# gitshitou/aclswarm

Measured on AMD Instinct MI355X. Metric: swarm assignment+control solves/sec (N=100) at 1/2/4/8 MI355X; % HBM roofline, higher is better.
Workload: dtype f64

## Files before the change

aclswarm_amd/_lib.py:

```python
import ctypes as ct
import os

import numpy as np

LIB_PATH = os.environ.get("ACLSWARM_AMD_LIB") or os.path.join(
    os.path.dirname(os.path.abspath(__file__)), "lib", "libaclswarm_amd.so")

ACL_OK = 0

FLAG_VALID = 0x01
FLAG_AGREE = 0x02
FLAG_CHANGED = 0x04
FLAG_NONFINITE = 0x08
FLAG_BAD_INPUT = 0x10
FLAG_CA_ACTIVE = 0x20
ABI_VERSION = 11
FLAG_FRAGILE = 0x40
FRAGILE_MARGIN = 1e-6

STATUS_DTYPE = np.dtype([("flags", "<u4"), ("eff_rounds", "<u2"),
                         ("rounds", "<u2"), ("n_invalid", "<u2"),
                         ("n_ca", "<u2"), ("margin", "<f4")])

EXPORTS = (
# ... 118 lines not shown
    _fields_ = [("B", ct.c_int32), ("fidx", ct.c_void_p), ("q", ct.c_void_p),
                ("vel", ct.c_void_p), ("P", ct.c_void_p), ("flush", ct.c_void_p),
                ("est", ct.c_void_p), ("ring_u", ct.c_void_p), ("ring_ca", ct.c_void_p),
                ("step0", ct.c_int32), ("steps", ct.c_int32), ("q_hist", ct.c_void_p),
                ("vel_hist", ct.c_void_p), ("u_hist", ct.c_void_p), ("ca_hist", ct.c_void_p), ("P_hist", ct.c_void_p),
                ("workspace", ct.c_void_p), ("cntrl", CntrlGains), ("safety", SafetyParams),
                ("ep", EpisodeParams)]


class TrialParams(ct.Structure):
    _fields_ = [("ep", EpisodeParams), ("tick_rate", ct.c_int32), ("settle_steps", ct.c_int32),
                ("hover_wait", ct.c_double), ("assignment_timeout", ct.c_double),
                ("formation_received_wait", ct.c_double), ("converged_wait", ct.c_double),
                ("gridlock_timeout", ct.c_double), ("trial_timeout", ct.c_double),
                ("alpha", ct.c_double)]


TRIAL_HOVERING, TRIAL_WAITING, TRIAL_FLYING, TRIAL_IN_FORMATION = 3, 4, 5, 6
TRIAL_GRIDLOCK, TRIAL_COMPLETE, TRIAL_TERMINATE = 7, 8, 9

TRIAL_STATUS_DTYPE = np.dtype([(k, "<i4") for k in (
    "state", "last_state", "timer_ticks", "formation", "ticks", "received", "logging",
    "commit", "next_auction", "conv_len", "conv_head", "grid_len", "grid_head", "log_init",
    "t_start", "t_grid", "done_step")] + [("n_auctions", "<u2"), ("n_invalid", "<u2"),
                                          ("n_skipped", "<u2"), ("n_disagree", "<u2"),
                                          ("per_vehicle", "<i4")])


class TrialArgs(ct.Structure):
    _fields_ = [("B", ct.c_int32), ("K", ct.c_int32)] + [
        (k, ct.c_void_p) for k in ("fseq", "fidx", "q", "vel", "P", "flush", "ts", "ctl_on",
                                   "ring_u", "ring_ca", "posf", "dist", "t_conv", "t_avoid",
                                   "n_assign")] + [
        ("step0", ct.c_int32), ("steps", ct.c_int32)] + [
        (k, ct.c_void_p) for k in ("q_hist", "vel_hist", "u_hist", "ca_hist", "ctl_hist",
                                   "P_hist", "state_hist", "workspace")] + [
        ("cntrl", CntrlGains), ("safety", SafetyParams), ("tp", TrialParams)]


HUNG_BAD_INPUT = 0x01
HUNG_NONFINITE = 0x02
HUNG_CMP_INVALID = 0x04

_lib = None


def lib():
    global _lib
    if _lib is not None:
        return _lib
    if not os.path.exists(LIB_PATH):
        raise RuntimeError(
            f"aclswarm_amd: native library {LIB_PATH} is missing. Build it with "
            "`python -m aclswarm_amd.build` (hipcc --offload-arch=gfx950).")
    import torch
    L = ct.CDLL(LIB_PATH)
    VP, I32, I64, SZ = ct.c_void_p, ct.c_int32, ct.c_int64, ct.c_size_t
    L.acl_default_cntrl_gains.argtypes = [ct.POINTER(CntrlGains)]
    L.acl_default_safety_params.argtypes = [ct.POINTER(SafetyParams)]
    L.acl_default_admm_params.argtypes = [ct.POINTER(AdmmParams)]
    L.acl_formations_init.argtypes = [ct.POINTER(Formations), I32, I32]
    L.acl_formations_init.restype = None
    L.acl_max_vehicles.restype = I32
    L.acl_abi_version.restype = I32
    if L.acl_abi_version() != ABI_VERSION:
        raise RuntimeError(f"aclswarm_amd: {LIB_PATH} has ABI {L.acl_abi_version()}, this "
                           f"package expects {ABI_VERSION}: rebuild (python -m aclswarm_amd.build)")
    L.acl_solve_workspace_bytes.argtypes = [I32, I32]
    L.acl_solve_workspace_bytes.restype = ct.c_size_t
    L.acl_solve_batch.argtypes = [ct.POINTER(Formations), ct.POINTER(SolveArgs), VP]
    L.acl_solve_batch.restype = ct.c_int
    L.acl_count_edges.argtypes = [I32, VP]
    L.acl_count_edges.restype = I64
    L.acl_pack_adjacency.argtypes = [I32, VP, VP]
    L.acl_pack_adjacency.restype = ct.c_int
    L.acl_pack_gains.argtypes = [I32, VP, VP, VP]
    L.acl_pack_gains.restype = ct.c_int
    L.acl_gain_planes.argtypes = [I32, VP, VP]
    L.acl_gain_planes.restype = I32
    L.acl_pack_gains_planes.argtypes = [I32, VP, VP, I32, VP]
    L.acl_pack_gains_planes.restype = ct.c_int
    L.acl_tile_gains.argtypes = [ct.POINTER(Formations), VP, VP]
    L.acl_swarm_stats.argtypes = [VP, I32, VP, VP, VP]
    L.acl_swarm_stats.restype = I32
    L.acl_tile_gains.restype = ct.c_int
    L.acl_admm_solve_batch.argtypes = [I32, I32, VP, VP, VP, VP, ct.POINTER(AdmmParams), VP]
    L.acl_admm_solve_batch.restype = ct.c_int
    L.acl_control_batch.argtypes = [ct.POINTER(Formations), ct.POINTER(ControlArgs), VP]
    L.acl_control_batch.restype = ct.c_int
    L.acl_default_episode_params.argtypes = [ct.POINTER(EpisodeParams)]
    L.acl_default_episode_params.restype = None
    L.acl_episode_workspace_bytes.argtypes = [I32, I32]
    L.acl_episode_workspace_bytes.restype = SZ
    L.acl_episode_batch.argtypes = [ct.POINTER(Formations), ct.POINTER(EpisodeArgs), VP]
    L.acl_episode_batch.restype = ct.c_int
    L.acl_default_trial_params.argtypes = [ct.POINTER(TrialParams)]
    L.acl_default_trial_params.restype = None
    L.acl_trial_workspace_bytes.argtypes = [I32, I32]
    L.acl_trial_workspace_bytes.restype = SZ
    L.acl_trial_init.argtypes = [ct.POINTER(TrialArgs), I32, VP]
    L.acl_trial_init.restype = ct.c_int
    L.acl_trial_batch.argtypes = [ct.POINTER(Formations), ct.POINTER(TrialArgs), VP]
    L.acl_trial_batch.restype = ct.c_int
    L.acl_generate_formation_groups.argtypes = [I32, I32, VP, I32, ct.c_double, ct.c_double,
                                                ct.c_double, ct.c_double, I64, VP, VP, VP,
                                                VP, VP]
    L.acl_generate_formation_groups.restype = ct.c_int
    L.acl_hungarian_batch.argtypes = [ct.POINTER(Formations), ct.POINTER(HungarianArgs), VP]
    L.acl_hungarian_batch.restype = ct.c_int
    L.acl_cbaa_step_batch.argtypes = [ct.POINTER(Formations), ct.POINTER(CbaaStepArgs), VP]
    L.acl_cbaa_step_batch.restype = ct.c_int
    L.acl_vehicle_start_batch.argtypes = [ct.POINTER(Formations), ct.POINTER(VehicleStartArgs),
                                          VP]
    L.acl_vehicle_start_batch.restype = ct.c_int
    L.acl_fleet_workspace_bytes.argtypes = [I32, I32, I32]
    L.acl_fleet_workspace_bytes.restype = SZ
    L.acl_fleet_auction_batch.argtypes = [ct.POINTER(Formations), ct.POINTER(FleetAuctionArgs),
                                          VP]
    L.acl_fleet_auction_batch.restype = ct.c_int
    L.acl_write_assignment_log.argtypes = [ct.c_char_p, I32, VP, VP, VP, VP, VP, VP]
    L.acl_write_assignment_log.restype = ct.c_int
    L.acl_read_assignment_log.argtypes = [ct.c_char_p, ct.POINTER(I32), VP, VP, VP, VP, VP, VP]
    L.acl_read_assignment_log.restype = ct.c_int
    L.acl_device_count.restype = I32
    L.acl_set_device.argtypes = [I32]
    L.acl_set_device.restype = ct.c_int
    L.acl_malloc.argtypes = [ct.POINTER(VP), SZ]
    L.acl_malloc.restype = ct.c_int
    L.acl_free.argtypes = [VP]
    L.acl_free.restype = ct.c_int
    for fn in ("acl_memcpy_h2d", "acl_memcpy_d2h"):
        getattr(L, fn).argtypes = [VP, VP, SZ, VP]
        getattr(L, fn).restype = ct.c_int
    L.acl_memset.argtypes = [VP, ct.c_int, SZ, VP]
    L.acl_memset.restype = ct.c_int
    L.acl_stream_synchronize.argtypes = [VP]
    L.acl_stream_synchronize.restype = ct.c_int
    L.acl_last_error.restype = ct.c_char_p
    L.acl_internal_kernel_timing.argtypes = [ct.c_int]
    L.acl_internal_kernel_timing.restype = None
    L.acl_internal_kernel_times.argtypes = [ct.POINTER(ct.c_double), ct.POINTER(ct.c_int)]
    L.acl_internal_kernel_times.restype = ct.c_int
    L.acl_internal_admm_flop_counter.argtypes = [VP]
    L.acl_internal_admm_flop_counter.restype = None
    if hasattr(L, "acl_internal_admm_mem_cap"):
        L.acl_internal_admm_mem_cap.argtypes = [SZ]
        L.acl_internal_admm_mem_cap.restype = None
    L.acl_internal_psd_project.argtypes = [ct.c_int, ct.c_int, VP, ct.c_double, VP, ct.c_int,
                                           ct.POINTER(ct.c_int)]
    L.acl_internal_psd_project.restype = ct.c_int
    if hasattr(L, "acl_internal_price_sweep"):
        L.acl_internal_price_sweep.argtypes = [VP, VP, VP, ct.c_int]
        L.acl_internal_price_sweep.restype = ct.c_int
    _lib = L
    return L


def check(rc, what="aclswarm_amd"):
    if rc != ACL_OK:
        msg = lib().acl_last_error().decode(errors="replace")
        raise RuntimeError(f"{what} failed (code {rc}): {msg}")


def default_episode_params():
    e = EpisodeParams()
    lib().acl_default_episode_params(ct.byref(e))
    return e


def default_trial_params():
    t = TrialParams()
    lib().acl_default_trial_params(ct.byref(t))
    return t


def default_gains():
    g = CntrlGains()
    lib().acl_default_cntrl_gains(ct.byref(g))
    return g


def default_safety():
    s = SafetyParams()
    lib().acl_default_safety_params(ct.byref(s))
    return s


def default_admm_params():
    a = AdmmParams()
    lib().acl_default_admm_params(ct.byref(a))
    return a
```

aclswarm_amd/csrc/auction.hip:

```cpp
#include <hip/hip_runtime.h>
#include <stdint.h>

#include "../../include/aclswarm_amd.h"
#include "common.h"
#include "control_dev.h"
#include "control_params.h"
#include "pair_fused.h"
#include "umeyama_dev.h"

namespace acl_amd {

#ifndef ACL_AUCTION_LEVELS
#define ACL_AUCTION_LEVELS 4
#endif
constexpr int kAL = ACL_AUCTION_LEVELS;

__host__ __device__ inline int a16(int x) { return (x + 15) & ~15; }

struct ALayout {
  int C, pq, adjF, items;
  int A, p, qf, out;
  int T, TS;
  int vadj, Pin, Ptin, itm, valid, H, misc, dummy, W1, total;
};
// ... 1112 lines not shown
      P.P_out[(size_t)b * n + v] = (uint16_t)jj;
      validv[v] = valid0;
      if (jj != Pin[v]) misc[M_CHANGED] = 1;
    }
  } else {
    for (int v = wave; v < n; v += kAW) {
      const unsigned char* row = T + v * TS;
      bool ismine[NC];
#pragma unroll
      for (int c = 0; c < NC; ++c) {
        const int jj = lane + 64 * c;
        ismine[c] = (jj < n) && (row[jj] == v);
      }
      int mine = -1;
#pragma unroll
      for (int c = NC - 1; c >= 0; --c) {
        const unsigned long long mm = __ballot(ismine[c]);
        if (mm) mine = 64 * c + __ffsll((long long)mm) - 1;
      }
      const bool valid = row_valid(row) && mine >= 0;
      const int adopted = valid ? mine : Pin[v];
      if (lane == 0) {
        validv[v] = valid;
        if (!valid) atomicAdd(&misc[M_NINV], 1);
        if (adopted != Pin[v]) misc[M_CHANGED] = 1;
        P.P_out[(size_t)b * n + v] = (uint16_t)adopted;
      }
    }
  }
  if (P.who) {
    for (int k = tid; k < n * n; k += kAB) {
      const int v = k / n, jj = k - v * n;
      const int w = T[v * TS + jj];
      P.who[(size_t)b * n * n + k] = (w >= n) ? (uint16_t)0xFFFF : (uint16_t)w;
    }
  }
  __syncthreads();
  stamp_phase(P, b, tid, 5);

  const int ninv = misc[M_NINV];
  const bool allvalid = ninv == 0;
  const bool uniform = (allvalid && misc[M_AGREE]) || (ninv == n && !rowsm);
  const int ptv = (uniform && tid < n) ? (allvalid ? T[tid] : Ptin[tid]) : 0;
  {
    uint16_t* wsPt = reinterpret_cast<uint16_t*>(P.ws + P.W.pt) + (size_t)b * n;
    if (tid == 0) P.ws[P.W.mode + b] = uniform ? 0 : 1;
    if (uniform) {
      for (int jj = tid; jj < n; jj += kAB) wsPt[jj] = allvalid ? T[jj] : Ptin[jj];
    } else {
      uint16_t* rows = reinterpret_cast<uint16_t*>(P.ws + P.W.rows) + (size_t)b * n * n;
      for (int k = tid; k < n * n; k += kAB) {
        const int v = k / n, jj = k - v * n;
        rows[k] = validv[v] ? T[v * TS + jj]
                  : rowsm ? P.P_rows[(size_t)b * n * n + k] : Ptin[jj];
      }
      for (int v = tid; v < n; v += kAB) P.ws[P.W.vvalid + (size_t)b * n + v] = validv[v];
    }
    if (tid == 0) {
      acl_swarm_status_t st = {};
      uint32_t fl = 0;
      if (allvalid) fl |= ACL_SWARM_VALID;
      if (misc[M_AGREE]) fl |= ACL_SWARM_AGREE;
      if (misc[M_CHANGED]) fl |= ACL_SWARM_CHANGED;
      if (nonfinite) fl |= ACL_SWARM_NONFINITE;
      const double g = !MG ? -1.0 : nonfinite ? 0.0 : __longlong_as_double((long long)*margw);
      if (MG && g < ACL_FRAGILE_MARGIN) fl |= ACL_SWARM_FRAGILE;
      st.flags = fl;
      st.eff_rounds = (uint16_t)eff;
      st.rounds = (uint16_t)(2 * n);
      st.n_invalid = (uint16_t)ninv;
      st.margin = (float)g;
      P.status[b] = st;
    }
  }
  stamp_phase(P, b, tid, 6);

  if constexpr (FUSE) {
    if (!uniform) return;
#ifdef ACL_EXP_SKIP_GAIN
    return;
#endif
    __syncthreads();
    const FusedLayout GL = make_fused_layout(n, kAW);
    if (tid < n) reinterpret_cast<uint16_t*>(smem + GL.Pt)[tid] = (uint16_t)ptv;
    KCtlParams* pc = (KCtlParams*)((const __attribute__((address_space(4))) char*)
                                       __builtin_amdgcn_kernarg_segment_ptr() +
                                   offsetof(SolveParams, ctl));
    asm volatile("" : "+s"(pc));
    if (!ACL_FUSED_PREFETCH) fused_prefetch(*pc, b, f, tid, fpre);
    if (ACL_CTL_PRIO || ACL_CBAA_PRIO) __builtin_amdgcn_s_setprio(ACL_CTL_PRIO);
    pair_gain_fused<kAW, GM>(pc, b, f, smem, tid, kAB, fpre);
    stamp_phase(P, b, tid, 7);
  }
  stamp_rt(P, b, tid, kStampRt1);
}

__global__ void price_sweep_kernel(const double* x, float* fast, float* ieee, int m) {
  const int i = blockIdx.x * blockDim.x + threadIdx.x;
  if (i < m) {
    fast[i] = acl_price(x[i]);
    ieee[i] = (float)(1.0 / (sqrt(x[i]) + 1e-8));
  }
}

static int auction_lds(int n, bool fuse) {
  const int a = make_alayout(n).total;
  if (!fuse) return a;
  const int kAW = n <= 32 ? 2 : (n <= 64 ? 4 : 8);
  const int g = make_fused_layout(n, kAW).total;
  return a > g ? a : g;
}

template <bool FUSE, bool GM, bool MG>
static hipError_t launch_auction_t(const SolveParams& P, int nb, hipStream_t stream) {
  static PerDeviceOnce once;
  const hipError_t ea = once.run([] {
    for (const void* k : {(const void*)auction_kernel<1, 128, FUSE, GM, MG>,
                          (const void*)auction_kernel<1, 256, FUSE, GM, MG>,
                          (const void*)auction_kernel<2, 512, FUSE, GM, MG>}) {
      const hipError_t e =
          hipFuncSetAttribute(k, hipFuncAttributeMaxDynamicSharedMemorySize, 160 * 1024);
      if (e != hipSuccess) return e;
    }
    return hipSuccess;
  });
  if (ea != hipSuccess) return ea;
  if (P.n > 64)
    hipLaunchKernelGGL((align_kernel<2>), dim3(nb), dim3(64), make_align_layout(P.n).total, stream,
                       P);
  const int lds = auction_lds(P.n, FUSE);
  if (P.n <= 32)
    hipLaunchKernelGGL((auction_kernel<1, 128, FUSE, GM, MG>), dim3(nb), dim3(128), lds, stream, P);
  else if (P.n <= 64)
    hipLaunchKernelGGL((auction_kernel<1, 256, FUSE, GM, MG>), dim3(nb), dim3(256), lds, stream, P);
  else
    hipLaunchKernelGGL((auction_kernel<2, 512, FUSE, GM, MG>), dim3(nb), dim3(512), lds, stream, P);
  return hipGetLastError();
}

hipError_t launch_auction(const SolveParams& P, int nb, hipStream_t stream, bool fuse) {
  const bool mg = !P.skip_margin;
  if (!fuse)
    return mg ? launch_auction_t<false, false, true>(P, nb, stream)
              : launch_auction_t<false, false, false>(P, nb, stream);
  if (P.ctl.gate_margin)
    return mg ? launch_auction_t<true, true, true>(P, nb, stream)
              : launch_auction_t<true, true, false>(P, nb, stream);
  return mg ? launch_auction_t<true, false, true>(P, nb, stream)
            : launch_auction_t<true, false, false>(P, nb, stream);
}

}

extern "C" int acl_internal_price_sweep(const double* x, float* fast, float* ieee, int m) {
  if (m <= 0) return 0;
  hipLaunchKernelGGL(acl_amd::price_sweep_kernel, dim3((m + 255) / 256), dim3(256), 0, 0, x, fast,
                     ieee, m);
  return hipDeviceSynchronize() == hipSuccess ? 0 : 1;
}
```

aclswarm_amd/csrc/pair_fused.h:

```cpp
#pragma once

#include "control_dev.h"

#ifndef ACL_DIAG_NOPAIR
#define ACL_DIAG_NOPAIR 0
#endif
#ifndef ACL_DIAG_NOLOADS
#define ACL_DIAG_NOLOADS 0
#endif
#ifndef ACL_DIAG_NOLOOP
#define ACL_DIAG_NOLOOP 0
#endif

namespace acl_amd {

struct FusedLayout {
  int pt, adj, etab, rowb, Pt, Pinv, acc, atab, cst, nearb, clf, vel, flags, gmw, caw, total;
};

enum { FC_K1XY, FC_K2XY, FC_K1Z, FC_K2Z, FC_TXY, FC_TZ, FC_WIN, FC_THR2, FC_N };

__host__ __device__ inline FusedLayout make_fused_layout(int n, int kW) {
  const int nb = (n + 7) >> 3, R = 8 * nb;
  FusedLayout L;
  int o = 0;
  L.pt = o;    o = cal16(o + R * 64);
  L.adj = o;   o = cal16(o + R * 2 * 8);
  L.etab = o;  o = cal16(o + R * nb * 4);
  L.rowb = o;  o = cal16(o + (R + 1) * 4);
  L.Pt = o;    o = cal16(o + n * 2);
  L.Pinv = o;  o = cal16(o + n * 2);
  L.acc = o;   o = cal16(o + kW * R * 3 * 8);
  L.atab = o;  o = cal16(o + ACL_ATAB_N * 8);
  L.cst = o;   o = cal16(o + FC_N * 8);
  L.nearb = o; o = cal16(o + 4 * 4);
  L.clf = o;   o = cal16(o + R * 4);
  L.vel = o;   o = cal16(o + n * 24);
  L.flags = o; o = cal16(o + 4);
  L.gmw = o;   o = o + 8;
  L.caw = o;   o = cal16(o + 4);
  L.total = o;
  return L;
}

struct Rec5 {
  double a[5];
};

__device__ __forceinline__ void load_rec5(__amdgpu_buffer_rsrc_t grs, int voff, Rec5& R) {
  const auto r0 = __builtin_amdgcn_raw_buffer_load_b128(grs, voff, 0, 0);
  const auto r1 = __builtin_amdgcn_raw_buffer_load_b128(grs, voff, 16, 0);
  const auto r2 = __builtin_amdgcn_raw_buffer_load_b64(grs, voff, 32, 0);
  __builtin_memcpy(&R.a[0], &r0, 16);
  __builtin_memcpy(&R.a[2], &r1, 16);
  __builtin_memcpy(&R.a[4], &r2, 8);
}

constexpr unsigned long long kTileUpIncl = 0x80C0E0F0F8FCFEFFull;
constexpr unsigned long long kTileUpStrict = kTileUpIncl & ~0x8040201008040201ull;
constexpr unsigned long long kColLanes = 0x000000FF00FF00FFull;

__device__ __forceinline__ double f64_of(unsigned lo, unsigned hi) {
  return __longlong_as_double((long long)(((unsigned long long)hi << 32) | lo));
}

__device__ __forceinline__ double col3_neg(double a, double b, double c3) {
  const unsigned long long ua = (unsigned long long)__double_as_longlong(a);
  const unsigned long long ub = (unsigned long long)__double_as_longlong(b);
  const auto s0 = __builtin_amdgcn_permlane32_swap((unsigned)ua, (unsigned)ub, false, false);
  const auto s1 = __builtin_amdgcn_permlane32_swap((unsigned)(ua >> 32), (unsigned)(ub >> 32),
                                                   false, false);
  const double p = f64_of(s0[0], s1[0]) + f64_of(s0[1], s1[1]);
  const double cc = swap_sum<32>(c3);
  const unsigned long long up = (unsigned long long)__double_as_longlong(p);
  const unsigned long long uc = (unsigned long long)__double_as_longlong(cc);
  const auto t0 = __builtin_amdgcn_permlane16_swap((unsigned)up, (unsigned)uc, false, false);
  const auto t1 = __builtin_amdgcn_permlane16_swap((unsigned)(up >> 32), (unsigned)(uc >> 32),
                                                   false, false);
  const double qn = -(f64_of(t0[0], t1[0]) + f64_of(t0[1], t1[1]));
  return qn + dpp_f64_all<0x128>(qn);
}

__device__ __forceinline__ double fcst(const double* cst, int k) {
  return *((const volatile __attribute__((address_space(3))) double*)(cst) + k);
}

typedef const __attribute__((address_space(4))) CtlParams KCtlParams;

__device__ __forceinline__ acl_cntrl_gains_t kgains(KCtlParams& P) {
  acl_cntrl_gains_t g;
  g.K1_xy = P.g.K1_xy; g.K2_xy = P.g.K2_xy; g.K1_z = P.g.K1_z; g.K2_z = P.g.K2_z;
  g.e_xy_thr = P.g.e_xy_thr; g.e_z_thr = P.g.e_z_thr; g.kp = P.g.kp; g.kd = P.g.kd;
  return g;
}

__device__ __forceinline__ acl_safety_params_t ksafety(KCtlParams& P) {
  acl_safety_params_t s;
  s.max_vel_xy = P.s.max_vel_xy; s.max_vel_z = P.s.max_vel_z;
  s.d_avoid_thresh = P.s.d_avoid_thresh; s.r_keep_out = P.s.r_keep_out;
  return s;
}

struct FusedPre {
  double q0, q1, q2, v0, v1, v2, px, py, pz;
  unsigned long long a0, a1;
};

__device__ __forceinline__ void fused_prefetch(KCtlParams& P, int b, int f, int tid,
                                               FusedPre& X) {
  const int n = P.n;
  X.q0 = X.q1 = X.q2 = X.v0 = X.v1 = X.v2 = X.px = X.py = X.pz = 0.0;
  X.a0 = X.a1 = 0ull;
  if (tid < n) {
    const int NWg = (n + 63) >> 6;
    const unsigned long long lastmask = (n & 63) ? ((1ull << (n & 63)) - 1ull) : ~0ull;
    const double* gq = P.q + ((size_t)b * n + tid) * 3;
    const double* gv = P.vel + ((size_t)b * n + tid) * 3;
    const double* gp = P.p + ((size_t)f * n + tid) * 3;
    const uint64_t* ga = P.adj + ((size_t)f * n + tid) * NWg;
    X.q0 = gq[0]; X.q1 = gq[1]; X.q2 = gq[2];
    X.v0 = gv[0]; X.v1 = gv[1]; X.v2 = gv[2];
    X.px = gp[0]; X.py = gp[1]; X.pz = gp[2];
    X.a0 = ga[0];
    if (NWg > 1) X.a1 = ga[1] & lastmask;
    else X.a0 &= lastmask;
  }
}

template <int kW, bool GM>
__device__ __forceinline__ void pair_gain_fused(KCtlParams* Pp, int b, int f,
                                                unsigned char* smem, int tid, int nthreads,
                                                const FusedPre& X) {
  KCtlParams& P = *Pp;
  const int n = P.n;
  const int nb = (n + 7) >> 3, R = 8 * nb;
  const FusedLayout L = make_fused_layout(n, kW);
  const int lane = tid & 63;
  const int wave = __builtin_amdgcn_readfirstlane(tid >> 6);

  double* pt = reinterpret_cast<double*>(smem + L.pt);
  unsigned long long* adjF = reinterpret_cast<unsigned long long*>(smem + L.adj);
  unsigned* etab = reinterpret_cast<unsigned*>(smem + L.etab);
  int* rowb = reinterpret_cast<int*>(smem + L.rowb);
  const uint16_t* Pt = reinterpret_cast<const uint16_t*>(smem + L.Pt);
  uint16_t* Pinv = reinterpret_cast<uint16_t*>(smem + L.Pinv);
  double* acc = reinterpret_cast<double*>(smem + L.acc);
  double* atab = reinterpret_cast<double*>(smem + L.atab);
  double* cst = reinterpret_cast<double*>(smem + L.cst);
  unsigned* nearb = reinterpret_cast<unsigned*>(smem + L.nearb);
  unsigned* clf = reinterpret_cast<unsigned*>(smem + L.clf);
  double* velv = reinterpret_cast<double*>(smem + L.vel);
  unsigned* flags = reinterpret_cast<unsigned*>(smem + L.flags);
  unsigned long long& gmw = *reinterpret_cast<unsigned long long*>(smem + L.gmw);
  unsigned* caw = reinterpret_cast<unsigned*>(smem + L.caw);
  double* qs = acc;

  for (int k = tid; k < ACL_ATAB_N; k += nthreads) atab[k] = ACL_ATAB_AT(k);
  if (GM && tid == 0) gmw = (unsigned long long)__double_as_longlong(__builtin_inf());
  if (tid == 0) {
    *caw = 0u;
    *flags = 0u;
  }
  if (tid < 4) nearb[tid] = 0u;
  for (int k = tid; k < R; k += nthreads) clf[k] = 0u;
  if (tid < FC_N) {
    const double thr_hi = P.s.d_avoid_thresh * (1.0 + 0x1p-40);
    const double v[FC_N] = {P.g.K1_xy, P.g.K2_xy, P.g.K1_z, P.g.K2_z,
                            P.g.e_xy_thr, P.g.e_z_thr, ACL_GATE_WINDOW, thr_hi * thr_hi};
    double x = v[0];
#pragma unroll
    for (int k = 1; k < FC_N; ++k) x = tid == k ? v[k] : x;
    cst[tid] = x;
  }
  {
    bool qbad = false;
    if (tid < n) {
      const int v = tid;
      qs[3 * v] = X.q0;
      qs[3 * v + 1] = X.q1;
      qs[3 * v + 2] = X.q2;
      velv[3 * v] = X.v0;
      velv[3 * v + 1] = X.v1;
      velv[3 * v + 2] = X.v2;
      qbad = !(__builtin_isfinite(X.q0) && __builtin_isfinite(X.q1) && __builtin_isfinite(X.q2));
    }
    if (tid < R) {
      const int i = tid;
      double row[5] = {0.0, 0.0, 0.0, 0.0, 0.0};
      if (i < n) {
        Pinv[Pt[i]] = (uint16_t)i;
        const double x = X.px, y = X.py, z = X.pz;
        row[0] = x;
        row[1] = y;
        row[2] = z;
        row[3] = x * x + y * y;
        row[4] = z * z;
      }
      pt[8 * i + 3] = row[0];
      reinterpret_cast<double4*>(pt + 8 * i)[1] = make_double4(row[1], row[2], row[3], row[4]);
      adjF[2 * i] = X.a0;
      adjF[2 * i + 1] = X.a1;
    }
    if (__any(qbad) && lane == 0) atomicOr(flags, 1u);
  }
  __syncthreads();
  if (tid < R) {
    const int i = tid;
    double q0 = 0.0, q1 = 0.0, q2 = 0.0;
    if (i < n) {
      const int v = Pt[i];
      q0 = qs[3 * v];
      q1 = qs[3 * v + 1];
      q2 = qs[3 * v + 2];
    }
    pt[8 * i] = q0;
    pt[8 * i + 1] = q1;
    pt[8 * i + 2] = q2;
  }
  if (wave == 0) {
    int base = 0;
    for (int i0 = 0; i0 < R; i0 += 64) {
      const int i = i0 + lane;
      const int cnt = (i < R) ? __popcll(adjF[2 * i]) + __popcll(adjF[2 * i + 1]) : 0;
      int x = cnt;
      x += __builtin_amdgcn_update_dpp(0, x, 0x111, 0xF, 0xF, true);
      x += __builtin_amdgcn_update_dpp(0, x, 0x112, 0xF, 0xF, true);
      x += __builtin_amdgcn_update_dpp(0, x, 0x114, 0xF, 0xF, true);
      x += __builtin_amdgcn_update_dpp(0, x, 0x118, 0xF, 0xF, true);
      x += __builtin_amdgcn_update_dpp(0, x, 0x142, 0xA, 0xF, false);
      x += __builtin_amdgcn_update_dpp(0, x, 0x143, 0xC, 0xF, false);
      if (i < R) rowb[i] = base + x - cnt;
      base += __builtin_amdgcn_readlane(x, 63);
    }
    if (lane == 0) rowb[R] = base;
  }
  __syncthreads();
  const unsigned nbm = (65536u + (unsigned)nb - 1u) / (unsigned)nb;
  for (int k = tid; k < R * nb; k += nthreads) {
    const int i = (int)(((unsigned)k * nbm) >> 16), J = k - i * nb;
    const int w = J >> 3, sh = (8 * J) & 63;
    const unsigned long long word = adjF[2 * i + w];
    const unsigned below = (unsigned)__popcll(sh ? (word & ((1ull << sh) - 1ull)) : 0ull) +
                           (w ? (unsigned)__popcll(adjF[2 * i]) : 0u);
    etab[k] = ((unsigned)rowb[i] + below) << 8 | (unsigned)((word >> sh) & 0xFFull);
  }
  for (int k = tid; k < kW * R * 3; k += nthreads) acc[k] = 0.0;
  const bool qfin = (*flags & 1u) == 0u;
  __syncthreads();

  double gmxy = __builtin_inf(), gmz = __builtin_inf();
  if (wave < kW) {
    const int E = __builtin_amdgcn_readfirstlane(rowb[R]);
    const double* G = P.gains + 5 * P.gain_off[f];
    const __amdgpu_buffer_rsrc_t grs =
        __builtin_amdgcn_make_buffer_rsrc((void*)G, (short)0, 5 * E * 8, 0x00020000);
    const int r = lane >> 3, c = lane & 7;
    const int colk = 3 * c + ((lane >> 4) == 0 ? 0 : ((lane >> 4) == 1 ? 2 : 1));
    const int NT = nb * (nb + 1) / 2;
    const int t0 = (wave * NT) / kW, t1 = ACL_DIAG_NOLOOP ? t0 : ((wave + 1) * NT) / kW;
    double* myacc = acc + wave * R * 3;

    int I = 0, J = 0;
    if (t0 < t1) {
      int rem = t0;
      while (rem >= nb - I) {
        rem -= nb - I;
        ++I;
      }
      J = I + rem;
    }
    auto rec_mask = [&](unsigned x, int s, bool diag, unsigned long long up) {
      return __ballot((x >> s) & 1u) & (diag ? up : ~0ull);
    };
    auto rec_load = [&](unsigned x, int s, unsigned long long m, Rec5& R) {
      const unsigned e = (x >> 8) + (unsigned)__popc(x & ((1u << s) - 1u));
#if ACL_DIAG_NOLOADS
      const double d = (double)(lanebit_u64(m) ? (e & 7u) : 0u) * 0.125;
      R.a[0] = d; R.a[1] = -d; R.a[2] = d; R.a[3] = d; R.a[4] = -d;
#else
      load_rec5(grs, lanebit_u64(m) ? (int)__umul24(e, 40u) : 0x40000000, R);
#endif
    };
    Rec5 X, Y;
    unsigned long long mx = 0ull, my = 0ull;
    if (t0 < t1) {
      const unsigned xij = etab[__umul24(8 * I + r, nb) + J], xji = etab[__umul24(8 * J + c, nb) + I];
      mx = rec_mask(xij, c, I == J, kTileUpIncl);
      my = rec_mask(xji, r, I == J, kTileUpStrict);
      rec_load(xij, c, mx, X);
      rec_load(xji, r, my, Y);
    }
    double ra0 = 0.0, ra1 = 0.0, ra2 = 0.0;
#pragma unroll 1
    for (int t = t0; t < t1; ++t) {
#pragma clang fp contract(fast)
      int In = I, Jn = J;
      if (++Jn == nb) {
        ++In;
        Jn = In;
      }
      const bool more = t + 1 < t1;
      unsigned xijn = 0u, xjin = 0u;
      if (more) {
        xijn = etab[__umul24(8 * In + r, nb) + Jn];
        xjin = etab[__umul24(8 * Jn + c, nb) + In];
      }
      const int i = 8 * I + r, j = 8 * J + c;
      const double4* pi = reinterpret_cast<const double4*>(pt + 8 * i);
      const double4* pj = reinterpret_cast<const double4*>(pt + 8 * j);
      const double4 ai = pi[0], aj = pj[0];
      const double q0 = aj.x - ai.x, q1 = aj.y - ai.y, q2 = aj.z - ai.z;
      const double s2 = pair_s2(q0, q1);
      {
        const int nr = n - 8 * I, nc = n - 8 * J;
        const unsigned long long rows = nr >= 8 ? ~0ull : ((1ull << (8 * nr)) - 1ull);
        const unsigned long long cols =
            (nc >= 8 ? 0xFFull : ((1ull << nc) - 1ull)) * 0x0101010101010101ull;
        const unsigned long long vm = rows & cols & (I == J ? kTileUpStrict : ~0ull);
        const unsigned long long nm = __ballot(!(s2 > fcst(cst, FC_THR2))) & vm;
        if (nm) {
          if (lanebit_u64(nm)) {
            atomicOr(&nearb[i >> 5], 1u << (i & 31));
            atomicOr(&nearb[j >> 5], 1u << (j & 31));
          }
        }
      }
      const unsigned long long many = mx | my;
      double Fxy = 0.0, Fz = 0.0;
      if (!ACL_DIAG_NOPAIR && lanebit_u64(many)) {
        const double4 bi = pi[1], bj = pj[1];
        const double pix = ai.w, piy = bi.x, piz = bi.y, pjx = aj.w, pjy = bj.x, pjz = bj.y;
        double e_xy, e_z;
        pair_e(q0, q1, q2, bi.z, bj.z, bi.w, bj.w, pix, piy, piz, pjx, pjy, pjz, s2, e_xy, e_z);
        bool gxy, gz;
        gate_decide_t<GM>(fcst(cst, FC_TXY), fcst(cst, FC_TZ), fcst(cst, FC_WIN), e_xy, e_z, q0,
                          q1, q2, bi.z, bj.z, bi.w, bj.w, pix, piy, piz, pjx, pjy, pjz, gxy, gz,
                          gmxy, gmz);
#if ACL_DIAG_NOATAN
        if (gxy) Fxy = fcst(cst, FC_K1XY) * (fcst(cst, FC_K2XY) * e_xy);
        if (gz) Fz = fcst(cst, FC_K1Z) * (fcst(cst, FC_K2Z) * e_z);
#else
        if (gxy) Fxy = fcst(cst, FC_K1XY) * ACL_GAIN_ATAN(fcst(cst, FC_K2XY) * e_xy, atab);
        if (gz) Fz = fcst(cst, FC_K1Z) * ACL_GAIN_ATAN(fcst(cst, FC_K2Z) * e_z, atab);
#endif
      }
      const double f0 = Fxy * q0, f1 = Fxy * q1, f2 = Fz * q2;
      if (lanebit_u64(mx)) {
        if (qfin) {
          ra0 += X.a[1] * q1 + (X.a[0] * q0 + f0);
          ra1 += X.a[3] * q1 + (X.a[2] * q0 + f1);
          ra2 += X.a[4] * q2 + f2;
        } else {
          ra0 += ((X.a[0] * q0 + X.a[1] * q1) + 0.0 * q2) + f0;
          ra1 += ((X.a[2] * q0 + X.a[3] * q1) + 0.0 * q2) + f1;
          ra2 += ((0.0 * q0 + 0.0 * q1) + X.a[4] * q2) + f2;
        }
      }
      unsigned long long mxn = 0ull, myn = 0ull;
      if (more) {
        mxn = rec_mask(xijn, c, In == Jn, kTileUpIncl);
        rec_load(xijn, c, mxn, X);
      }
      double ct0 = 0.0, ct1 = 0.0, ct2 = 0.0;
      if (lanebit_u64(my)) {
        if (qfin) {
          ct0 = Y.a[1] * q1 + (Y.a[0] * q0 + f0);
          ct1 = Y.a[3] * q1 + (Y.a[2] * q0 + f1);
          ct2 = Y.a[4] * q2 + f2;
        } else {
          ct0 = ((Y.a[0] * q0 + Y.a[1] * q1) + 0.0 * q2) + f0;
          ct1 = ((Y.a[2] * q0 + Y.a[3] * q1) + 0.0 * q2) + f1;
          ct2 = ((0.0 * q0 + 0.0 * q1) + Y.a[4] * q2) + f2;
        }
      }
      if (more) {
        myn = rec_mask(xjin, r, In == Jn, kTileUpStrict);
        rec_load(xjin, r, myn, Y);
      }
      {
        const double cs = col3_neg(ct0, ct1, ct2);
        if (lanebit_u64(kColLanes)) unsafeAtomicAdd(myacc + 24 * J + colk, cs);
      }
      if (!more || In != I) {
        ra0 += dpp_f64_all<0xB1>(ra0); ra1 += dpp_f64_all<0xB1>(ra1); ra2 += dpp_f64_all<0xB1>(ra2);
        ra0 += dpp_f64_all<0x4E>(ra0); ra1 += dpp_f64_all<0x4E>(ra1); ra2 += dpp_f64_all<0x4E>(ra2);
        ra0 += dpp_f64_all<0x141>(ra0); ra1 += dpp_f64_all<0x141>(ra1); ra2 += dpp_f64_all<0x141>(ra2);
        if (c == 0) {
          double* a = myacc + 3 * i;
          unsafeAtomicAdd(a, ra0);
          unsafeAtomicAdd(a + 1, ra1);
          unsafeAtomicAdd(a + 2, ra2);
        }
        ra0 = ra1 = ra2 = 0.0;
      }
      I = In;
      J = Jn;
      mx = mxn;
      my = myn;
    }
    if (GM) {
      const acl_cntrl_gains_t g = kgains(P);
      gate_margin_reduce(&gmw, gate_margin_of(g, gmxy, gmz));
    }
  }
  __syncthreads();
  if (GM && tid == 0) P.gate_margin[b] = __longlong_as_double((long long)gmw);
  if (nearb[0] | nearb[1] | nearb[2] | nearb[3]) {
    const double thr = P.s.d_avoid_thresh;
    const double thr_hi = thr * (1.0 + 0x1p-40);
    const double thr2hi = thr_hi * thr_hi;
    const int per = nthreads / n;
    const int v = tid % n, j0 = tid / n;
    if (j0 < per) {
      const int i = Pinv[v];
      if ((nearb[i >> 5] >> (i & 31)) & 1u) {
        const double qv0 = pt[8 * i], qv1 = pt[8 * i + 1];
        bool c = false;
        for (int k = j0; k < n; k += per) {
          const double dx = pt[8 * k] - qv0, dy = pt[8 * k + 1] - qv1;
          const double d2 = dx * dx + dy * dy;
          if (k != i && !(d2 > thr2hi)) c |= !(sqrt(d2) > thr);
        }
        if (c) clf[v] = 1u;
      }
    }
    __syncthreads();
  }

  {
    const acl_cntrl_gains_t g = kgains(P);
    const acl_safety_params_t sp = ksafety(P);
    const int NW = (n + 63) >> 6;
    for (int v = tid; v < n; v += nthreads) {
      const int i = Pinv[v];
      const int deg = __popcll(adjF[2 * i]) + __popcll(adjF[2 * i + 1]);
      double s0 = 0.0, s1 = 0.0, s2 = 0.0;
      for (int w = 0; w < kW; ++w) {
        const double* a = acc + (w * R + i) * 3;
        s0 += a[0];
        s1 += a[1];
        s2 += a[2];
      }
      double cmd0 = g.kp * s0, cmd1 = g.kp * s1, cmd2 = g.kp * s2;
      if (deg) {
        const double* gv = velv + 3 * v;
        const double cn = (double)deg;
        cmd0 += cn * (g.kd * (-gv[0]));
        cmd1 += cn * (g.kd * (-gv[1]));
        cmd2 += cn * (g.kd * (-gv[2]));
      }
      double* gu = P.u + ((size_t)b * n + v) * 3;
      gu[0] = cmd0;
      gu[1] = cmd1;
      gu[2] = cmd2;
      saturate(sp, cmd0, cmd1, cmd2);
      const bool close = clf[v] != 0u;
      if (P.u_safe) {
        double* o = P.u_safe + ((size_t)b * n + v) * 3;
        o[0] = cmd0;
        o[1] = cmd1;
        o[2] = cmd2;
      }
      if (P.ca_flag) P.ca_flag[(size_t)b * n + v] = 0;
      const unsigned long long cm = __ballot(close);
      if ((tid & 63) == 0) {
        P.ca_mask[(size_t)b * NW + (v >> 6)] = cm;
        if (cm && atomicOr(caw, 1u) == 0u) P.ca_list[atomicAdd(P.ca_count, 1u)] = (unsigned)b;
      }
    }
  }
}

}
```

Measured before the change: 7.846 million.

## Pack diagonal and ragged-edge tiles into full waves in fused pair loop

```diff
diff --git a/aclswarm_amd/_lib.py b/aclswarm_amd/_lib.py
--- a/aclswarm_amd/_lib.py
+++ b/aclswarm_amd/_lib.py
@@ -294,6 +294,11 @@
     if hasattr(L, "acl_internal_price_sweep"):
         L.acl_internal_price_sweep.argtypes = [VP, VP, VP, ct.c_int]
         L.acl_internal_price_sweep.restype = ct.c_int
+    if hasattr(L, "acl_internal_fused_tile_pairs"):
+        L.acl_internal_fused_tile_pairs.argtypes = [ct.c_int, ct.c_int, VP, ct.c_int]
+        L.acl_internal_fused_tile_pairs.restype = ct.c_int
+        L.acl_internal_fused_tile_counts.argtypes = [ct.c_int, ct.c_int, VP]
+        L.acl_internal_fused_tile_counts.restype = ct.c_int
     _lib = L
     return L
 
diff --git a/aclswarm_amd/csrc/auction.hip b/aclswarm_amd/csrc/auction.hip
--- a/aclswarm_amd/csrc/auction.hip
+++ b/aclswarm_amd/csrc/auction.hip
@@ -1288,6 +1288,50 @@
 
 }
 
+extern "C" int acl_internal_fused_tile_pairs(int n, int kW, int* out, int cap) {
+  using namespace acl_amd;
+  if (n < 1 || n > 128 || kW < 1 || kW > 8) return -1;
+  const FusedSched S = make_fused_sched(n);
+  int cnt = 0;
+  for (int wave = 0; wave < kW; ++wave) {
+    const FusedRange W = fused_wave_range(S, kW, wave);
+    const int tiles = (W.r1 - W.r0) + W.sn;
+    if (!tiles) continue;
+    int g = fused_wave_tile(S, W, 0);
+    FusedTile T = fused_tile_at(S, g);
+    for (int k = 0; k < tiles; ++k) {
+      for (int lane = 0; lane < 64; ++lane) {
+        int i, j;
+        bool valid;
+        fused_tile_lane(n, S.nb, T, lane, i, j, valid);
+        if (!valid) continue;
+        if (out && cnt < cap) {
+          int* o = out + 5 * (size_t)cnt;
+          o[0] = wave; o[1] = k; o[2] = lane; o[3] = i; o[4] = j;
+        }
+        ++cnt;
+      }
+      if (k + 1 < tiles) {
+        const int gn = fused_wave_tile(S, W, k + 1);
+        T = fused_tile_step(S, T, g, gn);
+        g = gn;
+      }
+    }
+  }
+  return cnt;
+}
+
+extern "C" int acl_internal_fused_tile_counts(int n, int kW, int* per_wave) {
+  using namespace acl_amd;
+  if (n < 1 || n > 128 || kW < 1 || kW > 8) return -1;
+  const FusedSched S = make_fused_sched(n);
+  for (int wave = 0; wave < kW; ++wave) {
+    const FusedRange W = fused_wave_range(S, kW, wave);
+    if (per_wave) per_wave[wave] = (W.r1 - W.r0) + W.sn;
+  }
+  return S.total;
+}
+
 extern "C" int acl_internal_price_sweep(const double* x, float* fast, float* ieee, int m) {
   if (m <= 0) return 0;
   hipLaunchKernelGGL(acl_amd::price_sweep_kernel, dim3((m + 255) / 256), dim3(256), 0, 0, x, fast,
diff --git a/aclswarm_amd/csrc/pair_fused.h b/aclswarm_amd/csrc/pair_fused.h
--- a/aclswarm_amd/csrc/pair_fused.h
+++ b/aclswarm_amd/csrc/pair_fused.h
@@ -43,6 +43,137 @@
   return L;
 }
 
+enum { FT_IJ = 0, FT_DIAG2 = 1, FT_FOLD = 2 };
+
+struct FusedSched {
+  int nb;
+  int nbr;
+  int nreg;
+  int xfold;
+  int xdiag;
+  int nij;
+  int ndiag2;
+  int nfold;
+  int total;
+};
+
+struct FusedTile {
+  int kind, a, b;
+};
+
+struct FusedRange {
+  int r0, r1, s0, sn, ss;
+};
+
+#ifndef ACL_FUSED_FOLD
+#define ACL_FUSED_FOLD 1
+#endif
+#ifndef ACL_FUSED_DIAG2
+#define ACL_FUSED_DIAG2 1
+#endif
+
+__host__ __device__ inline FusedSched make_fused_sched(int n) {
+  FusedSched S;
+  const int nb = (n + 7) >> 3, rem = n & 7;
+  const bool fold = ACL_FUSED_FOLD && rem >= 1 && rem <= 4;
+  S.nb = nb;
+  S.nbr = fold ? nb - 1 : nb;
+  S.nreg = S.nbr * (S.nbr - 1) / 2;
+  S.nfold = fold ? (nb - 1) >> 1 : 0;
+  S.xfold = fold ? (nb - 1) & 1 : 0;
+  S.ndiag2 = ACL_FUSED_DIAG2 ? nb >> 1 : 0;
+  S.xdiag = nb - 2 * S.ndiag2;
+  S.nij = S.nreg + S.xfold + S.xdiag;
+  S.total = S.nij + S.ndiag2 + S.nfold;
+  return S;
+}
+
+__host__ __device__ inline FusedRange fused_wave_range(const FusedSched& S, int kW, int wave) {
+  const int ns = S.ndiag2 + S.nfold;
+  const int A = S.total / kW, e = S.total - A * kW, a = ns / kW, b = ns - a * kW;
+  const int share = A + (wave < e ? 1 : 0), cs = a + (wave < b ? 1 : 0);
+  const int t0 = wave * A + (wave < e ? wave : e);
+  const int sp = wave * a + (wave < b ? wave : b);
+  FusedRange W;
+  W.r0 = t0 - sp;
+  W.r1 = W.r0 + share - cs;
+  W.s0 = wave;
+  W.sn = cs;
+  W.ss = kW;
+  return W;
+}
+
+__host__ __device__ inline int fused_wave_tile(const FusedSched& S, const FusedRange& W, int k) {
+  const int nr = W.r1 - W.r0;
+  return k < nr ? W.r0 + k : S.nij + W.s0 + (k - nr) * W.ss;
+}
+
+__host__ __device__ inline FusedTile fused_tile_at(const FusedSched& S, int g) {
+  FusedTile T;
+  if (g < S.nreg) {
+    int rem = g, a = 0;
+    while (rem >= S.nbr - 1 - a) {
+      rem -= S.nbr - 1 - a;
+      ++a;
+    }
+    T.kind = FT_IJ; T.a = a; T.b = a + 1 + rem;
+    return T;
+  }
+  g -= S.nreg;
+  if (g < S.xfold) {
+    T.kind = FT_IJ; T.a = S.nb - 2; T.b = S.nb - 1;
+    return T;
+  }
+  g -= S.xfold;
+  if (g < S.xdiag) {
+    T.kind = FT_IJ; T.a = T.b = S.nb - S.xdiag + g;
+    return T;
+  }
+  g -= S.xdiag;
+  if (g < S.ndiag2) {
+    T.kind = FT_DIAG2; T.a = 2 * g; T.b = 2 * g + 1;
+    return T;
+  }
+  g -= S.ndiag2;
+  T.kind = FT_FOLD; T.a = 2 * g; T.b = 2 * g + 1;
+  return T;
+}
+
+__host__ __device__ inline FusedTile fused_tile_step(const FusedSched& S, FusedTile T, int g,
+                                                     int gn) {
+  if (gn == g + 1 && gn < S.nreg) {
+    if (++T.b == S.nbr) {
+      ++T.a;
+      T.b = T.a + 1;
+    }
+    return T;
+  }
+  return fused_tile_at(S, gn);
+}
+
+__host__ __device__ inline void fused_lane_ij(int a, int b, int lane, int& i, int& j) {
+  i = 8 * a + (lane >> 3);
+  j = 8 * b + (lane & 7);
+}
+
+__host__ __device__ inline void fused_tile_lane(int n, int nb, const FusedTile& T, int lane,
+                                                int& i, int& j, bool& valid) {
+  const int r = lane >> 3, c = lane & 7;
+  if (T.kind == FT_IJ) {
+    fused_lane_ij(T.a, T.b, lane, i, j);
+    valid = i < n && j < n && (T.a != T.b || r < c);
+  } else if (T.kind == FT_DIAG2) {
+    const bool up = r < c;
+    i = up ? 8 * T.a + r : 8 * T.b + c;
+    j = up ? 8 * T.a + c : 8 * T.b + r;
+    valid = r != c && j < n;
+  } else {
+    i = 8 * T.a + (lane >> 2);
+    j = 8 * (nb - 1) + (lane & 3);
+    valid = j < n;
+  }
+}
+
 struct Rec5 {
   double a[5];
 };
@@ -256,19 +387,14 @@
         __builtin_amdgcn_make_buffer_rsrc((void*)G, (short)0, 5 * E * 8, 0x00020000);
     const int r = lane >> 3, c = lane & 7;
     const int colk = 3 * c + ((lane >> 4) == 0 ? 0 : ((lane >> 4) == 1 ? 2 : 1));
-    const int NT = nb * (nb + 1) / 2;
-    const int t0 = (wave * NT) / kW, t1 = ACL_DIAG_NOLOOP ? t0 : ((wave + 1) * NT) / kW;
+    const FusedSched S = make_fused_sched(n);
+    const FusedRange W = fused_wave_range(S, kW, wave);
+    const int nr = ACL_DIAG_NOLOOP ? 0 : W.r1 - W.r0;
+    const int cnt = ACL_DIAG_NOLOOP ? 0 : nr + W.sn;
     double* myacc = acc + wave * R * 3;
-
-    int I = 0, J = 0;
-    if (t0 < t1) {
-      int rem = t0;
-      while (rem >= nb - I) {
-        rem -= nb - I;
-        ++I;
-      }
-      J = I + rem;
-    }
+    int g = fused_wave_tile(S, W, 0);
+    FusedTile T = fused_tile_at(S, cnt ? g : 0);
+
     auto rec_mask = [&](unsigned x, int s, bool diag, unsigned long long up) {
       return __ballot((x >> s) & 1u) & (diag ? up : ~0ull);
     };
@@ -281,42 +407,52 @@
       load_rec5(grs, lanebit_u64(m) ? (int)__umul24(e, 40u) : 0x40000000, R);
 #endif
     };
-    Rec5 X, Y;
-    unsigned long long mx = 0ull, my = 0ull;
-    if (t0 < t1) {
-      const unsigned xij = etab[__umul24(8 * I + r, nb) + J], xji = etab[__umul24(8 * J + c, nb) + I];
-      mx = rec_mask(xij, c, I == J, kTileUpIncl);
-      my = rec_mask(xji, r, I == J, kTileUpStrict);
-      rec_load(xij, c, mx, X);
-      rec_load(xji, r, my, Y);
-    }
-    double ra0 = 0.0, ra1 = 0.0, ra2 = 0.0;
-#pragma unroll 1
-    for (int t = t0; t < t1; ++t) {
+    auto opaque_lane = [&]() {
+      int l = lane;
+      asm volatile("" : "+v"(l));
+      return l;
+    };
+    auto tile_words = [&](const FusedTile& N, unsigned& xij, unsigned& xji) {
+      if (N.kind == FT_IJ) {
+        xij = etab[__umul24(8 * N.a + r, nb) + N.b];
+        xji = etab[__umul24(8 * N.b + c, nb) + N.a];
+      } else {
+        int i, j;
+        bool v;
+        fused_tile_lane(n, nb, N, opaque_lane(), i, j, v);
+        xij = etab[__umul24(i, nb) + (j >> 3)];
+        xji = etab[__umul24(j, nb) + (i >> 3)];
+      }
+    };
+    auto tile_load = [&](const FusedTile& N, unsigned x, bool second, Rec5& R) {
+      unsigned long long m;
+      if (N.kind == FT_IJ) {
+        int s = second ? r : c;
+        asm volatile("" : "+v"(s));
+        m = rec_mask(x, s, N.a == N.b, second ? kTileUpStrict : kTileUpIncl);
+        rec_load(x, s, m, R);
+      } else {
+        int i, j;
+        bool v;
+        fused_tile_lane(n, nb, N, opaque_lane(), i, j, v);
+        const int s = (second ? i : j) & 7;
+        m = __ballot(v && ((x >> s) & 1u));
+        rec_load(x, s, m, R);
+      }
+      return m;
+    };
+    auto pair_eval = [&](int i, int j, unsigned long long vm, unsigned long long many,
+                         double& q0, double& q1, double& q2, double& f0, double& f1,
+                         double& f2) {
 #pragma clang fp contract(fast)
-      int In = I, Jn = J;
-      if (++Jn == nb) {
-        ++In;
-        Jn = In;
-      }
-      const bool more = t + 1 < t1;
-      unsigned xijn = 0u, xjin = 0u;
-      if (more) {
-        xijn = etab[__umul24(8 * In + r, nb) + Jn];
-        xjin = etab[__umul24(8 * Jn + c, nb) + In];
-      }
-      const int i = 8 * I + r, j = 8 * J + c;
       const double4* pi = reinterpret_cast<const double4*>(pt + 8 * i);
       const double4* pj = reinterpret_cast<const double4*>(pt + 8 * j);
       const double4 ai = pi[0], aj = pj[0];
-      const double q0 = aj.x - ai.x, q1 = aj.y - ai.y, q2 = aj.z - ai.z;
+      q0 = aj.x - ai.x;
+      q1 = aj.y - ai.y;
+      q2 = aj.z - ai.z;
       const double s2 = pair_s2(q0, q1);
       {
-        const int nr = n - 8 * I, nc = n - 8 * J;
-        const unsigned long long rows = nr >= 8 ? ~0ull : ((1ull << (8 * nr)) - 1ull);
-        const unsigned long long cols =
-            (nc >= 8 ? 0xFFull : ((1ull << nc) - 1ull)) * 0x0101010101010101ull;
-        const unsigned long long vm = rows & cols & (I == J ? kTileUpStrict : ~0ull);
         const unsigned long long nm = __ballot(!(s2 > fcst(cst, FC_THR2))) & vm;
         if (nm) {
           if (lanebit_u64(nm)) {
@@ -325,7 +461,6 @@
           }
         }
       }
-      const unsigned long long many = mx | my;
       double Fxy = 0.0, Fz = 0.0;
       if (!ACL_DIAG_NOPAIR && lanebit_u64(many)) {
         const double4 bi = pi[1], bj = pj[1];
@@ -344,44 +479,69 @@
         if (gz) Fz = fcst(cst, FC_K1Z) * ACL_GAIN_ATAN(fcst(cst, FC_K2Z) * e_z, atab);
 #endif
       }
-      const double f0 = Fxy * q0, f1 = Fxy * q1, f2 = Fz * q2;
+      f0 = Fxy * q0;
+      f1 = Fxy * q1;
+      f2 = Fz * q2;
+    };
+    auto rec_term = [&](const Rec5& A, double q0, double q1, double q2, double f0, double f1,
+                        double f2, double& t0, double& t1, double& t2) {
+#pragma clang fp contract(fast)
+      if (qfin) {
+        t0 = A.a[1] * q1 + (A.a[0] * q0 + f0);
+        t1 = A.a[3] * q1 + (A.a[2] * q0 + f1);
+        t2 = A.a[4] * q2 + f2;
+      } else {
+        t0 = ((A.a[0] * q0 + A.a[1] * q1) + 0.0 * q2) + f0;
+        t1 = ((A.a[2] * q0 + A.a[3] * q1) + 0.0 * q2) + f1;
+        t2 = ((0.0 * q0 + 0.0 * q1) + A.a[4] * q2) + f2;
+      }
+    };
+
+    Rec5 X, Y;
+    unsigned long long mx = 0ull, my = 0ull;
+    if (cnt) {
+      unsigned xij, xji;
+      tile_words(T, xij, xji);
+      mx = tile_load(T, xij, false, X);
+      my = tile_load(T, xji, true, Y);
+    }
+    int k = 0;
+    double ra0 = 0.0, ra1 = 0.0, ra2 = 0.0;
+#pragma unroll 1
+    for (; k < nr; ++k) {
+#pragma clang fp contract(fast)
+      const bool more = k + 1 < cnt;
+      const int gn = more ? fused_wave_tile(S, W, k + 1) : g;
+      const FusedTile Tn = more ? fused_tile_step(S, T, g, gn) : T;
+      unsigned xijn = 0u, xjin = 0u;
+      if (more) tile_words(Tn, xijn, xjin);
+      const int I = T.a, J = T.b;
+      int i, j;
+      fused_lane_ij(I, J, lane, i, j);
+      const int rn = n - 8 * I, cn = n - 8 * J;
+      const unsigned long long rows = rn >= 8 ? ~0ull : ((1ull << (8 * rn)) - 1ull);
+      const unsigned long long cols =
+          (cn >= 8 ? 0xFFull : ((1ull << cn) - 1ull)) * 0x0101010101010101ull;
+      const unsigned long long vm = rows & cols & (I == J ? kTileUpStrict : ~0ull);
+      double q0, q1, q2, f0, f1, f2;
+      pair_eval(i, j, vm, mx | my, q0, q1, q2, f0, f1, f2);
       if (lanebit_u64(mx)) {
-        if (qfin) {
-          ra0 += X.a[1] * q1 + (X.a[0] * q0 + f0);
-          ra1 += X.a[3] * q1 + (X.a[2] * q0 + f1);
-          ra2 += X.a[4] * q2 + f2;
-        } else {
-          ra0 += ((X.a[0] * q0 + X.a[1] * q1) + 0.0 * q2) + f0;
-          ra1 += ((X.a[2] * q0 + X.a[3] * q1) + 0.0 * q2) + f1;
-          ra2 += ((0.0 * q0 + 0.0 * q1) + X.a[4] * q2) + f2;
-        }
+        double t0, t1, t2;
+        rec_term(X, q0, q1, q2, f0, f1, f2, t0, t1, t2);
+        ra0 += t0;
+        ra1 += t1;
+        ra2 += t2;
       }
       unsigned long long mxn = 0ull, myn = 0ull;
-      if (more) {
-        mxn = rec_mask(xijn, c, In == Jn, kTileUpIncl);
-        rec_load(xijn, c, mxn, X);
-      }
+      if (more) mxn = tile_load(Tn, xijn, false, X);
       double ct0 = 0.0, ct1 = 0.0, ct2 = 0.0;
-      if (lanebit_u64(my)) {
-        if (qfin) {
-          ct0 = Y.a[1] * q1 + (Y.a[0] * q0 + f0);
-          ct1 = Y.a[3] * q1 + (Y.a[2] * q0 + f1);
-          ct2 = Y.a[4] * q2 + f2;
-        } else {
-          ct0 = ((Y.a[0] * q0 + Y.a[1] * q1) + 0.0 * q2) + f0;
-          ct1 = ((Y.a[2] * q0 + Y.a[3] * q1) + 0.0 * q2) + f1;
-          ct2 = ((0.0 * q0 + 0.0 * q1) + Y.a[4] * q2) + f2;
-        }
-      }
-      if (more) {
-        myn = rec_mask(xjin, r, In == Jn, kTileUpStrict);
-        rec_load(xjin, r, myn, Y);
-      }
+      if (lanebit_u64(my)) rec_term(Y, q0, q1, q2, f0, f1, f2, ct0, ct1, ct2);
+      if (more) myn = tile_load(Tn, xjin, true, Y);
       {
         const double cs = col3_neg(ct0, ct1, ct2);
         if (lanebit_u64(kColLanes)) unsafeAtomicAdd(myacc + 24 * J + colk, cs);
       }
-      if (!more || In != I) {
+      if (k + 1 == nr || Tn.a != I) {
         ra0 += dpp_f64_all<0xB1>(ra0); ra1 += dpp_f64_all<0xB1>(ra1); ra2 += dpp_f64_all<0xB1>(ra2);
         ra0 += dpp_f64_all<0x4E>(ra0); ra1 += dpp_f64_all<0x4E>(ra1); ra2 += dpp_f64_all<0x4E>(ra2);
         ra0 += dpp_f64_all<0x141>(ra0); ra1 += dpp_f64_all<0x141>(ra1); ra2 += dpp_f64_all<0x141>(ra2);
@@ -393,8 +553,77 @@
         }
         ra0 = ra1 = ra2 = 0.0;
       }
-      I = In;
-      J = Jn;
+      T = Tn;
+      g = gn;
+      mx = mxn;
+      my = myn;
+    }
+#pragma unroll 1
+    for (; k < cnt; ++k) {
+#pragma clang fp contract(fast)
+      const bool more = k + 1 < cnt;
+      const int gn = more ? fused_wave_tile(S, W, k + 1) : g;
+      const FusedTile Tn = more ? fused_tile_step(S, T, g, gn) : T;
+      unsigned xijn = 0u, xjin = 0u;
+      if (more) tile_words(Tn, xijn, xjin);
+      const int sl = opaque_lane(), sr = sl >> 3, sc = sl & 7;
+      const int scolk = 3 * sc + ((sl >> 4) == 0 ? 0 : ((sl >> 4) == 1 ? 2 : 1));
+      int i, j;
+      bool valid;
+      fused_tile_lane(n, nb, T, sl, i, j, valid);
+      double q0, q1, q2, f0, f1, f2;
+      pair_eval(i, j, __ballot(valid), mx | my, q0, q1, q2, f0, f1, f2);
+      double rt0 = 0.0, rt1 = 0.0, rt2 = 0.0;
+      if (lanebit_u64(mx)) rec_term(X, q0, q1, q2, f0, f1, f2, rt0, rt1, rt2);
+      double ct0 = 0.0, ct1 = 0.0, ct2 = 0.0;
+      if (lanebit_u64(my)) rec_term(Y, q0, q1, q2, f0, f1, f2, ct0, ct1, ct2);
+      if (T.kind == FT_FOLD) {
+        rt0 += dpp_f64_all<0xB1>(rt0); rt1 += dpp_f64_all<0xB1>(rt1); rt2 += dpp_f64_all<0xB1>(rt2);
+        rt0 += dpp_f64_all<0x4E>(rt0); rt1 += dpp_f64_all<0x4E>(rt1); rt2 += dpp_f64_all<0x4E>(rt2);
+        if ((sl & 3) == 0) {
+          double* a = myacc + 3 * i;
+          unsafeAtomicAdd(a, rt0);
+          unsafeAtomicAdd(a + 1, rt1);
+          unsafeAtomicAdd(a + 2, rt2);
+        }
+        double cs = col3_neg(ct0, ct1, ct2);
+        cs += dpp_f64_all<0x124>(cs);
+        if (lanebit_u64(kColLanes & 0x0F0F0F0F0F0F0F0Full))
+          unsafeAtomicAdd(myacc + 24 * (nb - 1) + scolk, cs);
+      } else {
+        const bool up = sr < sc;
+        {
+          double a0 = up ? rt0 : 0.0, a1 = up ? rt1 : 0.0, a2 = up ? rt2 : 0.0;
+          double b0 = up ? 0.0 : ct0, b1 = up ? 0.0 : ct1, b2 = up ? 0.0 : ct2;
+          a0 += dpp_f64_all<0xB1>(a0); a1 += dpp_f64_all<0xB1>(a1); a2 += dpp_f64_all<0xB1>(a2);
+          b0 += dpp_f64_all<0xB1>(b0); b1 += dpp_f64_all<0xB1>(b1); b2 += dpp_f64_all<0xB1>(b2);
+          a0 += dpp_f64_all<0x4E>(a0); a1 += dpp_f64_all<0x4E>(a1); a2 += dpp_f64_all<0x4E>(a2);
+          b0 += dpp_f64_all<0x4E>(b0); b1 += dpp_f64_all<0x4E>(b1); b2 += dpp_f64_all<0x4E>(b2);
+          a0 += dpp_f64_all<0x141>(a0); a1 += dpp_f64_all<0x141>(a1); a2 += dpp_f64_all<0x141>(a2);
+          b0 += dpp_f64_all<0x141>(b0); b1 += dpp_f64_all<0x141>(b1); b2 += dpp_f64_all<0x141>(b2);
+          if (sc == 0) {
+            double* a = myacc + 3 * (8 * T.a + sr);
+            unsafeAtomicAdd(a, a0);
+            unsafeAtomicAdd(a + 1, a1);
+            unsafeAtomicAdd(a + 2, a2);
+            double* bb = myacc + 3 * (8 * T.b + sr);
+            unsafeAtomicAdd(bb, -b0);
+            unsafeAtomicAdd(bb + 1, -b1);
+            unsafeAtomicAdd(bb + 2, -b2);
+          }
+        }
+        const double ca = col3_neg(up ? ct0 : 0.0, up ? ct1 : 0.0, up ? ct2 : 0.0);
+        if (lanebit_u64(kColLanes)) unsafeAtomicAdd(myacc + 24 * T.a + scolk, ca);
+        const double cb = col3_neg(up ? 0.0 : -rt0, up ? 0.0 : -rt1, up ? 0.0 : -rt2);
+        if (lanebit_u64(kColLanes)) unsafeAtomicAdd(myacc + 24 * T.b + scolk, cb);
+      }
+      unsigned long long mxn = 0ull, myn = 0ull;
+      if (more) {
+        mxn = tile_load(Tn, xijn, false, X);
+        myn = tile_load(Tn, xjin, true, Y);
+      }
+      T = Tn;
+      g = gn;
       mx = mxn;
       my = myn;
     }
```

Result: no change. 7.877 million (median of 6 runs) (+0.4%).
